# aifoundry-org/MHAQ

Hardware: AMD Instinct MI355X
Metric: qat_images_per_sec (higher is better)
Workload: dtype f32; 1 GPU; ResNet-18 ImageNet-1k QAT step, AEWGS weights per-channel + STE activations, Sym-KL distillation from FP teacher, RAdam, synthetic 224x224, channels_last memory format; per_gpu_batch=250, global_batch=250, parallelism=dp1, sync_batchnorm=False, weight_backward_groups=3, cudnn_benchmark=False

## Files before the change

include/mhaq_fq.h:

```cpp
#ifndef MHAQ_FQ_H
#define MHAQ_FQ_H

#include <stddef.h>
#include <stdint.h>

#ifdef __cplusplus
extern "C" {
#endif

#define MHAQ_FQ_ABI_VERSION 4

enum { MHAQ_FQ_STE = 0, MHAQ_FQ_EWGS = 1, MHAQ_FQ_AEWGS = 2, MHAQ_FQ_LSQ = 3 };

enum {
  MHAQ_FQ_EINVAL = -1,
  MHAQ_FQ_EWORKSPACE = -2,
  MHAQ_FQ_EALIGN = -3,
  MHAQ_FQ_EUNSUPPORTED = -4
};

enum {
  MHAQ_FQ_FLAG_BELOW_MIN = 1,
  MHAQ_FQ_FLAG_ABOVE_MAX = 2,
  MHAQ_FQ_FLAG_NOT_INTEGER = 4
// ... 70 lines not shown
                                  const float* params , int method, uint64_t seed, uint64_t offset,
                                  const uint64_t* offset_dev, void* workspace, size_t workspace_bytes,
                                  int32_t* nparts_out, void* stream);

int mhaq_fq_act_relu_fwd_x16(const void* z, const void* addend, void* y, void* a_out, int64_t n, int dtype,
                             const float* log_act_s, const float* log_act_q, const float* act_b,
                             float* params_out , void* stream);
int mhaq_fq_act_relu_bwd_x16(const void* z, const void* g_y, const void* g_a, void* gx, int64_t n, int dtype,
                             const float* params , int method, uint64_t seed, uint64_t offset,
                             const uint64_t* offset_dev, float* grads , void* workspace,
                             size_t workspace_bytes, void* stream);
int mhaq_fq_act_relu_bwd_partials_x16(const void* z, const void* g_y, const void* g_a, void* gx, int64_t n, int dtype,
                                      const float* params , int method, uint64_t seed, uint64_t offset,
                                      const uint64_t* offset_dev, void* workspace, size_t workspace_bytes,
                                      int32_t* nparts_out, void* stream);

size_t mhaq_fq_bn_bwd_workspace_bytes(int64_t m, int64_t c);
int mhaq_fq_bn_bwd(const float* x, const float* dy, const float* mean, const float* invstd, const float* weight,
                   float* dx, float* dweight, float* dbias, int64_t m, int64_t c,
                   void* workspace, size_t workspace_bytes, void* stream);

size_t mhaq_fq_bn_fwd_workspace_bytes(int64_t m, int64_t c);
int mhaq_fq_bn_fwd(const float* x, const float* weight, const float* bias, float* y,
                   float* save_mean, float* save_invstd, float* running_mean, float* running_var,
                   double factor, double eps, int64_t m, int64_t c,
                   void* workspace, size_t workspace_bytes, void* stream);

size_t mhaq_fq_bn_bwd_x16_workspace_bytes(int64_t m, int64_t c);
int mhaq_fq_bn_bwd_x16(const void* x, const void* dy, const float* mean, const float* invstd, const float* weight,
                       void* dx, float* dweight, float* dbias, int64_t m, int64_t c, int dtype,
                       void* workspace, size_t workspace_bytes, void* stream);

int mhaq_fq_maxpool3s2_fwd(const float* t, float* p, uint8_t* code, int64_t n, int64_t h, int64_t w, int64_t c,
                           void* stream);
size_t mhaq_fq_bn_pool_bwd_workspace_bytes(int64_t n, int64_t h, int64_t w, int64_t c);
int mhaq_fq_bn_pool_bwd(const float* x, const float* g, const uint8_t* code, const float* mean, const float* invstd,
                        const float* weight, float* dx, float* dweight, float* dbias, int64_t n, int64_t h, int64_t w,
                        int64_t c, void* workspace, size_t workspace_bytes, void* stream);

int mhaq_fq_maxpool3s2_fwd_x16(const void* t, void* p, uint8_t* code, int64_t n, int64_t h, int64_t w, int64_t c, int dtype,
                               void* stream);
size_t mhaq_fq_bn_pool_bwd_x16_workspace_bytes(int64_t n, int64_t h, int64_t w, int64_t c);
int mhaq_fq_bn_pool_bwd_x16(const void* x, const void* g, const uint8_t* code, const float* mean, const float* invstd,
                            const float* weight, void* dx, float* dweight, float* dbias, int64_t n, int64_t h, int64_t w,
                            int64_t c, int dtype, void* workspace, size_t workspace_bytes, void* stream);

enum { MHAQ_FQ_BN_RELU = 0, MHAQ_FQ_BN_ADD_RELU = 1, MHAQ_FQ_BN2_ADD_RELU = 2 };
int mhaq_fq_bn_infer_consts(const float* running_mean, const float* running_var, const float* weight, const float* bias,
                            double eps, int64_t c, float* consts , void* stream);
int mhaq_fq_bn_infer_act(const float* x, const float* consts, const float* x2, const float* consts2, const float* residual,
                         float* y, int64_t m, int64_t c, int mode, void* stream);
int mhaq_fq_bn_relu_pool3s2(const float* x, const float* consts, float* p, int64_t n, int64_t h, int64_t w, int64_t c,
                            void* stream);

size_t mhaq_fq_minmax_workspace_bytes(int64_t n);
int mhaq_fq_minmax(const float* x, int64_t n, float* out ,
                   void* workspace, size_t workspace_bytes, void* stream);

int mhaq_fq_row_minmax(const float* w, int64_t co, int64_t row, float* mn_out ,
                       float* mx_out , void* stream);

int mhaq_fq_pt_tie_scatter(const float* w, float* gw, int64_t n, const float* zp,
                           const float* grads , void* stream);

size_t mhaq_fq_pt_aewgs_colstats_workspace_bytes(int64_t co, int64_t row);
int mhaq_fq_pt_aewgs_colstats(const float* w, const float* G, int64_t co, int64_t row,
                              const float* s, const float* zp, const float* lo, const float* hi,
                              float* stats, void* workspace, size_t workspace_bytes, void* stream);

int mhaq_fq_pc_fwd(const float* w, float* wq, float* zp_out , float* q_out ,
                   const float* s , int64_t co, int64_t row, void* stream);

int mhaq_fq_pc_bwd(const float* w, const float* G, float* gw, float* g_s ,
                   const float* s , const float* zp ,
                   int64_t co, int64_t row, int method, const float* stats,
                   const float* gzp_extra ,
                   const int8_t* r_sign, uint64_t seed, uint64_t offset, const uint64_t* offset_dev, void* stream);

int mhaq_fq_wlayer_fwd(const float* w, float* wq, const float* log_s , int64_t co, int64_t row,
                       float* s_out, float* zp_out, float* mx_out, float* lwq_out ,
                       void* stream);
int mhaq_fq_wlayer_bwd(const float* w, const float* G, float* gw, float* g_log_s ,
                       const float* s, const float* zp, const float* mx, const float* g_lwq ,
                       int64_t co, int64_t row, int method, const float* stats,
                       const float* gzp_extra, const int8_t* r_sign, uint64_t seed, uint64_t offset, const uint64_t* offset_dev,
                       void* stream);

int64_t mhaq_fq_wlayer_pt_max_elements(void);
int mhaq_fq_wlayer_pt_fwd(const float* w, float* wq, const float* log_s , int64_t n,
                          float* aux , void* stream);
int mhaq_fq_wlayer_pt_bwd(const float* w, const float* G, float* gw, float* g_log_s ,
                          const float* aux, const float* g_lwq, int64_t n, int method,
                          const int8_t* r_sign, uint64_t seed, uint64_t offset, const uint64_t* offset_dev, void* stream);

size_t mhaq_fq_wlayer_ptl_workspace_bytes(int64_t n);
int mhaq_fq_wlayer_ptl_fwd(const float* w, float* wq, const float* log_s , int64_t n, float* aux ,
                           void* workspace, size_t workspace_bytes, void* stream);
int mhaq_fq_wlayer_ptl_bwd(const float* w, const float* G, float* gw, float* g_log_s ,
                           const float* aux , const float* g_lwq , int64_t n, int method,
                           const float* col_stats, int64_t period,
                           const int8_t* r_sign, uint64_t seed, uint64_t offset, const uint64_t* offset_dev,
                           void* workspace, size_t workspace_bytes, void* stream);

typedef struct {
  const float* w;
  const float* log_s;
// ... 58 lines not shown
```

mhaq_amd/_lib.py:

```python
from __future__ import annotations

import ctypes as C
import os
import re

_HERE = os.path.dirname(os.path.abspath(__file__))
LIB_PATH = os.environ.get("MHAQ_FQ_LIB") or os.path.join(_HERE, "csrc", "libmhaq_fq.so")
HEADER_PATH = os.path.join(os.path.dirname(_HERE), "include", "mhaq_fq.h")

_p = C.c_void_p
_i64 = C.c_int64
_u64 = C.c_uint64
_sz = C.c_size_t
_int = C.c_int

DT_BF16 = 1
DT_F16 = 2

SIGNATURES = {
    "mhaq_fq_abi_version": (_int, []),
    "mhaq_fq_error_string": (C.c_char_p, [_int]),
    "mhaq_fq_fill_r": (_int, [_p, _i64, _u64, _u64, _p]),
    "mhaq_fq_pt_fwd_workspace_bytes": (_sz, [_i64]),
    "mhaq_fq_pt_fwd": (_int, [_p, _p, _i64, _p, _p, _p, _p, _p, _p, _p, _p, _sz, _p]),
    "mhaq_fq_pt_bwd_workspace_bytes": (_sz, [_i64]),
    "mhaq_fq_pt_bwd": (_int, [_p, _p, _p, _i64, _p, _p, _p, _p, _int, _p, _i64, _p, _u64, _u64, _p, _int, _p, _p, _sz, _p]),
    "mhaq_fq_pt_bwd_partials": (_int, [_p, _p, _p, _i64, _p, _p, _p, _p, _int, _p, _i64, _p, _u64, _u64, _p, _int, _p, _sz,
                                       _p, _p]),
    "mhaq_fq_pt_bwd_finalize": (_int, [_p, C.c_int32, _p, _p]),
    "mhaq_fq_act_fwd": (_int, [_p, _p, _i64, _p, _p, _p, _p, _p, _p, _p, _sz, _p]),
    "mhaq_fq_act_bwd_workspace_bytes": (_sz, [_i64]),
    "mhaq_fq_act_bwd": (_int, [_p, _p, _p, _i64, _p, _int, _p, _u64, _u64, _p, _p, _p, _sz, _p]),
    "mhaq_fq_act_bwd_partials": (_int, [_p, _p, _p, _i64, _p, _int, _p, _u64, _u64, _p, _p, _sz, _p, _p]),
    "mhaq_fq_act_bwd_finalize_multi": (_int, [_p, _int, _p, _p]),
    "mhaq_fq_act_fwd_x16": (_int, [_p, _p, _i64, _int, _p, _p, _p, _p, _p, _p, _p, _sz, _p]),
    "mhaq_fq_act_bwd_x16": (_int, [_p, _p, _p, _i64, _int, _p, _int, _p, _u64, _u64, _p, _p, _p, _sz, _p]),
    "mhaq_fq_act_bwd_partials_x16": (_int, [_p, _p, _p, _i64, _int, _p, _int, _p, _u64, _u64, _p, _p, _sz, _p, _p]),
    "mhaq_fq_act_relu_fwd": (_int, [_p, _p, _p, _p, _i64, _p, _p, _p, _p, _p]),
    "mhaq_fq_act_relu_bwd": (_int, [_p, _p, _p, _p, _i64, _p, _int, _u64, _u64, _p, _p, _p, _sz, _p]),
    "mhaq_fq_act_relu_bwd_partials": (_int, [_p, _p, _p, _p, _i64, _p, _int, _u64, _u64, _p, _p, _sz, _p, _p]),
    "mhaq_fq_act_relu_fwd_x16": (_int, [_p, _p, _p, _p, _i64, _int, _p, _p, _p, _p, _p]),
    "mhaq_fq_act_relu_bwd_x16": (_int, [_p, _p, _p, _p, _i64, _int, _p, _int, _u64, _u64, _p, _p, _p, _sz, _p]),
    "mhaq_fq_act_relu_bwd_partials_x16": (_int, [_p, _p, _p, _p, _i64, _int, _p, _int, _u64, _u64, _p, _p, _sz, _p, _p]),
    "mhaq_fq_bn_bwd_workspace_bytes": (_sz, [_i64, _i64]),
    "mhaq_fq_bn_bwd": (_int, [_p, _p, _p, _p, _p, _p, _p, _p, _i64, _i64, _p, _sz, _p]),
    "mhaq_fq_bn_fwd_workspace_bytes": (_sz, [_i64, _i64]),
    "mhaq_fq_bn_fwd": (_int, [_p, _p, _p, _p, _p, _p, _p, _p, C.c_double, C.c_double, _i64, _i64, _p, _sz, _p]),
    "mhaq_fq_bn_bwd_x16_workspace_bytes": (_sz, [_i64, _i64]),
    "mhaq_fq_bn_bwd_x16": (_int, [_p, _p, _p, _p, _p, _p, _p, _p, _i64, _i64, _int, _p, _sz, _p]),
    "mhaq_fq_maxpool3s2_fwd": (_int, [_p, _p, _p, _i64, _i64, _i64, _i64, _p]),
    "mhaq_fq_bn_pool_bwd_workspace_bytes": (_sz, [_i64, _i64, _i64, _i64]),
    "mhaq_fq_bn_pool_bwd": (_int, [_p, _p, _p, _p, _p, _p, _p, _p, _p, _i64, _i64, _i64, _i64, _p, _sz, _p]),
    "mhaq_fq_maxpool3s2_fwd_x16": (_int, [_p, _p, _p, _i64, _i64, _i64, _i64, _int, _p]),
    "mhaq_fq_bn_pool_bwd_x16_workspace_bytes": (_sz, [_i64, _i64, _i64, _i64]),
    "mhaq_fq_bn_pool_bwd_x16": (_int, [_p, _p, _p, _p, _p, _p, _p, _p, _p, _i64, _i64, _i64, _i64, _int, _p, _sz, _p]),
    "mhaq_fq_bn_infer_consts": (_int, [_p, _p, _p, _p, C.c_double, _i64, _p, _p]),
    "mhaq_fq_bn_infer_act": (_int, [_p, _p, _p, _p, _p, _p, _i64, _i64, _int, _p]),
    "mhaq_fq_bn_relu_pool3s2": (_int, [_p, _p, _p, _i64, _i64, _i64, _i64, _p]),
    "mhaq_fq_minmax_workspace_bytes": (_sz, [_i64]),
    "mhaq_fq_minmax": (_int, [_p, _i64, _p, _p, _sz, _p]),
    "mhaq_fq_row_minmax": (_int, [_p, _i64, _i64, _p, _p, _p]),
    "mhaq_fq_pt_tie_scatter": (_int, [_p, _p, _i64, _p, _p, _p]),
    "mhaq_fq_pt_aewgs_colstats_workspace_bytes": (C.c_size_t, [_i64, _i64]),
    "mhaq_fq_pt_aewgs_colstats": (_int, [_p, _p, _i64, _i64, _p, _p, _p, _p, _p, _p, C.c_size_t, _p]),
    "mhaq_fq_pc_fwd": (_int, [_p, _p, _p, _p, _p, _i64, _i64, _p]),
    "mhaq_fq_pc_bwd": (_int, [_p, _p, _p, _p, _p, _p, _i64, _i64, _int, _p, _p, _p, _u64, _u64, _p, _p]),
    "mhaq_fq_pc_aewgs_stats": (_int, [_p, _p, _p, _p, _i64, _i64, _p, _p]),
    "mhaq_fq_wlayer_fwd": (_int, [_p, _p, _p, _i64, _i64, _p, _p, _p, _p, _p]),
    "mhaq_fq_wlayer_bwd": (_int, [_p, _p, _p, _p, _p, _p, _p, _p, _i64, _i64, _int, _p, _p, _p, _u64, _u64, _p, _p]),
    "mhaq_fq_wlayer_fwd_multi": (_int, [_p, _int, _i64, _i64, _p, _p, _p]),
    "mhaq_fq_wlayer_bwd_multi": (_int, [_p, _int, _i64, _i64, _p, _p, _p, _int, _p, _u64, _u64, _p, _p]),
    "mhaq_fq_wlayer_bwd_group": (_int, [_p, _int, _i64, _i64, _p, _i64, _p, _p, _int, _p, _u64, _u64, _p, _p]),
    "mhaq_fq_wlayer_aewgs_stats_group": (_int, [_p, _int, _i64, _p, _i64, _p, _p]),
    "mhaq_fq_pc_quantize": (_int, [_p, _p, _p, _p, _p, _i64, _i64, _p, _p]),
    "mhaq_fq_wlayer_pt_max_elements": (_i64, []),
    "mhaq_fq_wlayer_pt_fwd": (_int, [_p, _p, _p, _i64, _p, _p]),
    "mhaq_fq_wlayer_pt_bwd": (_int, [_p, _p, _p, _p, _p, _p, _i64, _int, _p, _u64, _u64, _p, _p]),
    "mhaq_fq_wlayer_ptl_workspace_bytes": (_sz, [_i64]),
    "mhaq_fq_wlayer_ptl_fwd": (_int, [_p, _p, _p, _i64, _p, _p, _sz, _p]),
    "mhaq_fq_wlayer_ptl_bwd": (_int, [_p, _p, _p, _p, _p, _p, _i64, _int, _p, _i64, _p, _u64, _u64, _p, _p, _sz, _p]),
    "mhaq_fq_vec_fwd": (_int, [_p, _p, _p, _p, _p, _i64, _p]),
    "mhaq_fq_vec_aewgs_stats": (_int, [_p, _p, _p, _p, _i64, _p, _p]),
    "mhaq_fq_vec_bwd": (_int, [_p, _p, _p, _p, _p, _p, _p, _i64, _int, _p, _p, _u64, _u64, _p, _p]),
    "mhaq_fq_potential_loss_fwd": (_int, [_p, _p, _p, _i64, _p, _p, _i64, C.c_float, C.c_float, C.c_float, _int,
                                          _p, _int, _p, _p]),
    "mhaq_fq_potential_loss_bwd": (_int, [_p, _p, _p, _p, _i64, _p, _p, _i64, C.c_float, C.c_float, C.c_float,
                                          _p, _p, _p, _p, _p, _p]),
    "mhaq_fq_noise_fwd": (_int, [_p, _p, _i64, _p]),
    "mhaq_fq_noise_bwd_workspace_bytes": (_sz, [_i64, _i64]),
    "mhaq_fq_noise_bwd": (_int, [_p, _p, _p, _p, _i64, _i64, _int, _p, _i64, _p, _u64, _u64, _p, _p, _sz, _p]),
}

_lib = None


class MhaqFqError(RuntimeError):
    pass


def header_functions():
    with open(HEADER_PATH) as f:
        src = re.sub(r"/\*.*?\*/", "", f.read(), flags=re.S)
    return sorted(set(re.findall(r"\b(mhaq_fq_\w+)\s*\(", src)))


def _try_build() -> None:
    import fcntl
    import subprocess
    import sys
    csrc = os.path.dirname(LIB_PATH)
    with open(os.path.join(csrc, ".build.lock"), "w") as lock:
# ... 37 lines not shown
```

mhaq_amd/csrc/torch_binding.cpp:

```cpp
#include <torch/extension.h>
#include <torch/version.h>
#include <torch/csrc/autograd/custom_function.h>

#include <c10/hip/HIPCachingAllocator.h>
#include <c10/hip/HIPGraphsC10Utils.h>
#include <c10/hip/HIPStream.h>
#include <c10/core/DeviceGuard.h>
#include <dlfcn.h>

#include <algorithm>
#include <atomic>
#include <chrono>
#include <cstring>
#include <map>
#include <memory>
#include <mutex>
#include <string>
#include <unordered_map>
#include <vector>

#include "../../include/mhaq_fq.h"

namespace py = pybind11;
using at::Tensor;
using torch::autograd::AutogradContext;
using torch::autograd::variable_list;

namespace {

#define MHAQ_API(X)                                                                                                   \
  X(mhaq_fq_abi_version) X(mhaq_fq_error_string) X(mhaq_fq_act_fwd) X(mhaq_fq_act_bwd_workspace_bytes)                \
  X(mhaq_fq_act_bwd) X(mhaq_fq_act_bwd_partials) X(mhaq_fq_act_bwd_finalize_multi) X(mhaq_fq_wlayer_fwd)              \
  X(mhaq_fq_wlayer_bwd) X(mhaq_fq_pc_aewgs_stats) X(mhaq_fq_wlayer_fwd_multi) X(mhaq_fq_wlayer_bwd_group)             \
  X(mhaq_fq_wlayer_aewgs_stats_group) X(mhaq_fq_wlayer_pt_fwd) X(mhaq_fq_wlayer_pt_bwd)                               \
  X(mhaq_fq_potential_loss_fwd) X(mhaq_fq_potential_loss_bwd) X(mhaq_fq_wlayer_ptl_workspace_bytes)                   \
  X(mhaq_fq_wlayer_ptl_fwd) X(mhaq_fq_wlayer_ptl_bwd) X(mhaq_fq_pt_aewgs_colstats_workspace_bytes)                     \
  X(mhaq_fq_pt_aewgs_colstats) X(mhaq_fq_act_fwd_x16) X(mhaq_fq_act_bwd_x16) X(mhaq_fq_act_bwd_partials_x16)                    \
  X(mhaq_fq_act_relu_fwd) X(mhaq_fq_act_relu_bwd) X(mhaq_fq_act_relu_bwd_partials)                                    \
  X(mhaq_fq_act_relu_fwd_x16) X(mhaq_fq_act_relu_bwd_x16) X(mhaq_fq_act_relu_bwd_partials_x16)                        \
  X(mhaq_fq_bn_bwd_workspace_bytes) X(mhaq_fq_bn_bwd) X(mhaq_fq_maxpool3s2_fwd)                                       \
  X(mhaq_fq_bn_pool_bwd_workspace_bytes) X(mhaq_fq_bn_pool_bwd) X(mhaq_fq_bn_bwd_x16_workspace_bytes)                 \
  X(mhaq_fq_bn_bwd_x16) X(mhaq_fq_bn_fwd_workspace_bytes) X(mhaq_fq_bn_fwd)                                         \
  X(mhaq_fq_bn_infer_consts) X(mhaq_fq_bn_infer_act) X(mhaq_fq_bn_relu_pool3s2)

struct Api {
#define X(n) decltype(&::n) n = nullptr;
  MHAQ_API(X)
#undef X
  void* handle = nullptr;
  std::string path;
};
Api A;

struct MhaqError : std::runtime_error {
  using std::runtime_error::runtime_error;
};

void bind_library(const std::string& path) {
  if (A.handle && A.path == path) return;
  void* h = dlopen(path.c_str(), RTLD_NOW | RTLD_LOCAL);
  if (!h) throw MhaqError("cannot load " + path + ": " + dlerror() + " (there is no CPU fallback)");
  Api a;
#define X(n)                                                                        \
  a.n = reinterpret_cast<decltype(a.n)>(dlsym(h, #n));                              \
  if (!a.n) throw MhaqError(std::string(#n) + " is not exported by " + path);
  MHAQ_API(X)
#undef X
  if (a.mhaq_fq_abi_version() != MHAQ_FQ_ABI_VERSION) throw MhaqError("libmhaq_fq.so ABI version mismatch");
  a.handle = h;
  a.path = path;
  A = a;
}

inline void need_lib() {
  if (!A.handle) throw MhaqError("the C-ABI library is not bound (mhaq_amd._ext.bind)");
}

inline void check(int rc, const char* what) {
  if (rc != 0)
    throw MhaqError(std::string(what) + " failed: " + A.mhaq_fq_error_string(rc) + " (code " + std::to_string(rc) + ")");
}

inline void* cur_stream(const Tensor& t) {
  return (void*)c10::hip::getCurrentHIPStream(t.device().index()).stream();
}

inline bool capturing() {
  return c10::hip::currentStreamCaptureStatusMayInitCtx() != c10::hip::CaptureStatus::None;
}

#define MHAQ_ON_DEVICE_OF(t) const c10::OptionalDeviceGuard mhaq_device_guard_(at::device_of(t))

inline const float* fptr(const Tensor& t) { return static_cast<const float*>(t.const_data_ptr()); }
inline float* fptr_mut(const Tensor& t) { return static_cast<float*>(t.mutable_data_ptr()); }
inline const float* fptr_or_null(const Tensor& t) { return t.defined() ? fptr(t) : nullptr; }

// ... 1267 lines not shown
    Tensor lws = lws_in.reshape({-1}).contiguous(), lwq = lwq_in.reshape({-1}).contiguous();
    TORCH_CHECK(las.numel() == laq.numel() && lws.numel() == lwq.numel(),
                "potential_loss: scale and range vectors must pair up");
    Tensor out = at::empty({12}, base.options());
    check(A.mhaq_fq_potential_loss_fwd(fptr(base), fptr(las), fptr(laq), las.numel(), fptr(lws), fptr(lwq), lws.numel(),
                                       (float)a_bits, (float)w_bits, (float)p, lossless ? 1 : 0, fptr_mut(state),
                                       update_state ? 1 : 0, fptr_mut(out), cur_stream(base)),
          "mhaq_fq_potential_loss_fwd");
    ctx->save_for_backward({out, las, laq, lws, lwq});
    ctx->saved_data["a"] = a_bits;
    ctx->saved_data["w"] = w_bits;
    ctx->saved_data["p"] = p;
    ctx->mark_non_differentiable({out});
    return {out.select(0, 0).clone(), out};
  }

  static variable_list backward(AutogradContext* ctx, variable_list grads) {
    auto saved = ctx->get_saved_variables();
    const Tensor &out = saved[0], &las = saved[1], &laq = saved[2], &lws = saved[3], &lwq = saved[4];
    Tensor g = grads[0].reshape({1}).contiguous();
    const int64_t na = las.numel(), nw = lws.numel();
    Tensor slab = at::empty({1 + 2 * na + 2 * nw}, out.options());
    Tensor g_base = slab.narrow(0, 0, 1), g_las = slab.narrow(0, 1, na), g_laq = slab.narrow(0, 1 + na, na),
           g_lws = slab.narrow(0, 1 + 2 * na, nw), g_lwq = slab.narrow(0, 1 + 2 * na + nw, nw);
    check(A.mhaq_fq_potential_loss_bwd(fptr(g), fptr(out), fptr(las), fptr(laq), na, fptr(lws), fptr(lwq), nw,
                                       (float)ctx->saved_data["a"].toDouble(), (float)ctx->saved_data["w"].toDouble(),
                                       (float)ctx->saved_data["p"].toDouble(), fptr_mut(g_base), fptr_mut(g_las),
                                       fptr_mut(g_laq), fptr_mut(g_lws), fptr_mut(g_lwq), cur_stream(out)),
          "mhaq_fq_potential_loss_bwd");
    const auto shapes = ctx->saved_data["shapes"].to<std::vector<std::vector<int64_t>>>();
    variable_list res(11);
    res[0] = g_base.reshape(shapes[0]);
    res[1] = g_las.reshape(shapes[1]);
    res[2] = g_laq.reshape(shapes[2]);
    res[3] = g_lws.reshape(shapes[3]);
    res[4] = g_lwq.reshape(shapes[4]);
    return res;
  }
};

std::pair<Tensor, Tensor> potential_loss(const Tensor& base, const Tensor& las, const Tensor& laq, const Tensor& lws,
                                         const Tensor& lwq, const Tensor& state, double a_bits, double w_bits, double p,
                                         bool lossless, bool update_state) {
  need_lib();
  MHAQ_ON_DEVICE_OF(base);
  for (const Tensor* t : {&base, &las, &laq, &lws, &lwq})
    TORCH_CHECK(t->is_cuda() && t->scalar_type() == at::kFloat, "potential_loss: inputs must be float32 device tensors");
  TORCH_CHECK(state.is_cuda() && state.scalar_type() == at::kFloat && state.numel() == 3 && state.is_contiguous(),
              "potential_loss: state must be a contiguous float32 device tensor {loss_sum, cnt, t}");
  auto out = PotentialLossFn::apply(base, las, laq, lws, lwq, state, a_bits, w_bits, p, lossless, update_state);
  return {out[0], out[1]};
}

}

PYBIND11_MODULE(TORCH_EXTENSION_NAME, m) {
  m.doc() = "compiled autograd binding of the mhaq_amd fused layer ops over the C ABI of include/mhaq_fq.h";
  m.attr("TORCH_VERSION") = TORCH_VERSION;
  static PyObject* err_class = nullptr;
  py::register_exception_translator([](std::exception_ptr p) {
    try {
      if (p) std::rethrow_exception(p);
    } catch (const MhaqError& e) {
      PyErr_SetString(err_class ? err_class : PyExc_RuntimeError, e.what());
    }
  });
  m.def("bind", [](const std::string& path, py::object error_class) {
    if (!err_class) err_class = error_class.inc_ref().ptr();
    bind_library(path);
  }, "dlopen the C-ABI library and resolve the entry points the nodes call");
  m.def("host_timers", [](bool reset) {
    py::dict d;
    for (int i = 0; i < T_N; ++i) {
      const int64_t n = g_tcnt[i].load(), ns = g_tns[i].load();
      d[kTimerNames[i]] = py::make_tuple(n, n ? (double)ns / (double)n * 1e-3 : 0.0);
      if (reset) { g_tcnt[i].store(0); g_tns[i].store(0); }
    }
    return d;
  }, py::arg("reset") = true);
  m.def("bound_library", []() { return A.path; });

  m.def("rng_manual_seed", [](uint64_t seed) { std::lock_guard<std::mutex> g(R.mu); R.seed = seed; R.seeded = true; R.count = 0; });
  m.def("rng_seed", []() -> py::object { std::lock_guard<std::mutex> g(R.mu); return R.seeded ? py::object(py::int_(R.seed)) : py::none(); });
  m.def("rng_next", [](int64_t rank) {
    std::lock_guard<std::mutex> g(R.mu);
    if (!R.seeded) throw MhaqError("sign stream used before it was seeded");
    return std::make_pair(R.seed ^ ((uint64_t)rank * kGolden), ++R.count);
  });
  m.def("rng_drawn", []() { std::lock_guard<std::mutex> g(R.mu); return R.count; });
  m.def("rng_set_drawn", [](uint64_t n) { std::lock_guard<std::mutex> g(R.mu); R.count = n; });
  m.def("rng_set_base", [](const std::optional<Tensor>& base) {
    std::lock_guard<std::mutex> g(R.mu);
    R.base = (base.has_value() && base->defined()) ? *base : Tensor();
  });
  m.def("rng_base", []() -> std::optional<Tensor> {
    std::lock_guard<std::mutex> g(R.mu);
    return R.base.defined() ? std::optional<Tensor>(R.base) : std::nullopt;
  });

  m.def("set_allreduce_avg", [](py::object fn) {
    g_allreduce_avg = fn.is_none() ? nullptr : fn.inc_ref().ptr();
  });
  m.def("set_dist_active", [](bool v) { g_dist_active.store(v); });

  m.def("hub_create", &hub_create);
  m.def("hub_destroy", [](int64_t id) { g_hubs.erase(id); });
// ... 33 lines not shown
        "number of BatchNorm backwards so far that ran the 16-bit HIP kernels (mhaq_fq_bn_bwd_x16)");
  m.def("bn_pool_train", &bn_pool_train, py::arg("x"), py::arg("weight"), py::arg("bias"), py::arg("running_mean"),
        py::arg("running_var"), py::arg("momentum"), py::arg("eps"), py::arg("cudnn_enabled") = true,
        py::arg("hip_forward") = false);
  m.def("bn_pool_hip_backwards", []() { return g_bn_pool_hip_backwards.load(); },
        "number of BatchNorm + pool backwards so far that ran mhaq_fq_bn_pool_bwd (the fallback is the two separate nodes)");

  m.def("bn_infer_consts", &bn_infer_consts, py::arg("running_mean"), py::arg("running_var"), py::arg("weight"),
        py::arg("bias"), py::arg("eps"), py::arg("consts"));
  m.def("bn_infer_act", &bn_infer_act, py::arg("x"), py::arg("consts"), py::arg("mode"), py::arg("x2") = py::none(),
        py::arg("consts2") = py::none(), py::arg("residual") = py::none());
  m.def("bn_relu_pool", &bn_relu_pool, py::arg("x"), py::arg("consts"));
  m.def("teacher_fused_calls", []() { return g_teacher_fused_calls.load(); },
        "number of fused launches so far on a frozen network's elementwise chain (bn_infer_act and bn_relu_pool)");

  m.def("weight_layer", &weight_layer, py::arg("w"), py::arg("log_wght_s"), py::arg("method"),
        py::arg("r_sign") = py::none(), py::arg("zp_grad") = false, py::arg("pre") = py::none(), py::arg("rank") = 0);
  m.def("weight_layer_pt", &weight_layer_pt, py::arg("w"), py::arg("log_wght_s"), py::arg("method"),
        py::arg("r_sign") = py::none(), py::arg("rank") = 0);
  m.def("weight_layer_ptl", &weight_layer_ptl, py::arg("w"), py::arg("log_wght_s"), py::arg("method"),
        py::arg("r_sign") = py::none(), py::arg("rank") = 0);

  m.def("plan_create", &plan_create);
  m.def("plan_destroy", [](int64_t id) { g_plans.erase(id); });
  m.def("plan_forward", &plan_forward);
  m.def("plan_group_apply", &plan_group_apply);
  m.def("plan_release_captured", [](int64_t id) {
    auto p = g_plans.get(id);
    std::lock_guard<std::mutex> g(p->mu);
    for (auto& grp : p->groups) if (grp.pool) grp.pool->release_captured();
    p->fwd_tables.release_captured();
  });
  m.def("plan_state", [](int64_t id) {
    auto p = g_plans.get(id);
    std::lock_guard<std::mutex> g(p->mu);
    py::dict d;
    d["fwd_tables"] = p->fwd_tables.entries.size();
    py::list pools;
    for (auto& grp : p->groups) {
      py::dict e;
      size_t used = 0, held = 0, size = 0;
      if (grp.pool) {
        size = grp.pool->keys.size();
        for (size_t i = 0; i < size; ++i) { used += grp.pool->used[i]; held += grp.pool->held[i]; }
      }
      e["size"] = size; e["used"] = used; e["held"] = held;
      pools.append(e);
    }
    d["pools"] = pools;
    return d;
  });

  m.def("potential_loss", &potential_loss);
}
```

mhaq_amd/qat.py:

```python
from __future__ import annotations

import contextlib
import copy
import time
from dataclasses import dataclass, field
from typing import Optional

import torch
import torch.distributed as dist
from torch import nn

from . import ops
from ._lib import MhaqFqError
from .enums import QNMethod, QScheme
from .loss import FusedPotentialLoss, FusedPotentialLossNoPred, SymmetricalKL
from .wrap import get_model_values, quantize_model


@dataclass
class QATConfig:
    qscheme: QScheme = QScheme.PER_CHANNEL
    qnmethod: QNMethod = QNMethod.AEWGS
    act_bit: int = 1
    weight_bit: int = 1
    calib_act_bit: int = 10
    calib_weight_bit: int = 10
    excluded_layers: tuple = ("conv1", "fc")
    quantize_bias: bool = False
    distillation: bool = True
    learning_rate: float = 3e-4
    warmup: int = 100
    scale_lr: float = 1.0
    scale_t: float = 2.0
    sync_batchnorm: bool = True
    overlap_teacher: bool = True
    joint_act_finalize: bool = True
    student_high_priority: bool = False
    multi_weight_forward: bool = True
    weight_backward_group_elems: int = 4 << 20
    fuse_blocks: bool = True
    fuse_stem_pool: bool = True
    hip_bn_backward: bool = True
    hip_bn_backward_16bit: bool = False
    hip_bn_forward: bool = False
    fuse_teacher: bool = True
    criterion: nn.Module = field(default_factory=nn.CrossEntropyLoss)
    autocast_dtype: Optional[torch.dtype] = None


@torch.no_grad()
def calibrate_weights(model: nn.Module, wbits: int, max_bits: int = 24, row_minmax_fn=None) -> None:
    row_minmax_fn = row_minmax_fn or ops.row_minmax
    for m in model.modules():
        if hasattr(m, "log_wght_s") and hasattr(m, "weight"):
            mn, mx = row_minmax_fn(m.weight)
            mn, mx = mn.cpu(), mx.cpu()
            if m.log_wght_s.numel() == 1 and mn.numel() != 1:
                mn, mx = mn.min(), mx.max()
            if not m.log_wght_s.requires_grad:
                wbits = max_bits
            floor = torch.log2((mx - mn) / (2 ** wbits - 1)).reshape(m.log_wght_s.shape)
            m.log_wght_s.copy_(torch.max(m.log_wght_s.detach().cpu(), floor))


def _cpu_row_minmax(w):
    dims = tuple(range(1, w.dim()))
    return w.detach().amin(dims), w.detach().amax(dims)


@torch.no_grad()
def calibrate_activations(model: nn.Module, batches, abits: int, max_bits: int = 24, minmax_fn=None) -> None:
    minmax_fn = minmax_fn or ops.minmax
    acts = [m for m in model.modules() if hasattr(m, "log_act_s") and hasattr(m, "act_b")]
    seen = {id(a): [] for a in acts}
    hooks = [a.register_forward_pre_hook(lambda mod, inp: seen[id(mod)].append(minmax_fn(inp[0]))) for a in acts]
    was_training = model.training
    model.eval()
    for x in batches:
        model(x)
    for h in hooks:
        h.remove()
    model.train(was_training)
    for a in acts:
        mm = torch.stack(seen[id(a)]).cpu()
        mn, mx = mm[:, 0].min(), mm[:, 1].max()
        if not a.log_act_q.requires_grad and not a.log_act_s.requires_grad:
            abits = max_bits
        if mx - mn > 0:
            log_s = torch.log2((mx - mn) / (2 ** abits - 1))
            a.act_b.fill_(mn)
            a.log_act_s.fill_(log_s)
            a.log_act_q.fill_(log_s + abits)
        else:
            a.log_act_q.zero_(), a.log_act_s.zero_(), a.act_b.fill_(mn)
            a.log_act_q.requires_grad_(False), a.log_act_s.requires_grad_(False), a.act_b.requires_grad_(False)


class TemperatureSchedule:
# ... 112 lines not shown
                pass
        self.module = _QATModule(net, cfg.qscheme, self.act_hub, self.weight_forward)
        self._flat_sync = False
        want_capture = capture_graph
        if want_capture is None:
            want_capture = "auto" if (layers is None and optimizer_factory is None and not multi_tensor_weights) else False
        if self.distributed and want_capture and self.device.type == "cuda" and self.multi is None:
            step_collectives = any(isinstance(m, nn.SyncBatchNorm) for m in net.modules()) or any(
                ops._method_value(m.Q.qnmethod) == QNMethod.AEWGS.value for m in net.modules() if hasattr(m, "Q")
            ) or next(iter(net.buffers()), None) is not None
            self._flat_sync = not step_collectives
        if self.distributed:
            for p in [m.log_b_s for m in net.modules() if hasattr(m, "log_b_s")]:
                p.requires_grad_(False)
            if self._flat_sync:
                with torch.no_grad():
                    for t in list(net.parameters()) + list(net.buffers()):
                        dist.broadcast(t, 0)
            else:
                self._wrap_ddp()
        if loss_classes is None:
            if self.device.type != "cuda":
                raise MhaqFqError("QATTrainer on a CPU device needs loss_classes (and layers): the fake-quant path and "
                                  "its PotentialLoss run only as HIP kernels (no CPU fallback by design)")
            loss_classes = (FusedPotentialLoss, FusedPotentialLossNoPred)
        if cfg.distillation:
            self.loss = loss_classes[0](SymmetricalKL(), p=1, a=cfg.act_bit, w=cfg.weight_bit)
        else:
            self.loss = loss_classes[1](cfg.criterion, p=1, a=cfg.act_bit, w=cfg.weight_bit)
        if capture_graph is None:
            stock = layers is None and optimizer_factory is None and not multi_tensor_weights
            capture_graph = "auto" if stock else False
        self.capture_graph = capture_graph if capture_graph == "auto" else bool(capture_graph)
        self._graph = self._static = self._static_loss = None
        self._rng_base = None
        self._rng_host0 = self._rng_stride = 0
        self._preflight, self._preflight_syncs = False, []
        self._flat_cache = None
        self._eager_steps = 0
        self._host_share = []
        self._static_grads, self._grads_detached = [], False
        if self.capture_graph:
            if (self.distributed and not self._flat_sync) or self.device.type != "cuda" or self.multi is not None:
                if self.capture_graph == "auto":
                    self.capture_graph = False
                else:
                    raise ValueError("capture_graph needs a step without host code or collectives inside it: a "
                                     "single GPU, or data parallelism without SyncBatchNorm and without the AEWGS "
                                     "statistics exchange (then the gradients take one flat all-reduce after the "
                                     "replay); not the multi-tensor joint backward")
        if self.capture_graph:
            self._rng_base = torch.zeros(1, dtype=torch.int64, device=self.device)
            self._gstream = torch.cuda.Stream(device=self.device)
        self.optimizer = (optimizer_factory or torch.optim.RAdam)(self.net.parameters(), cfg.learning_rate)
        self.schedule = TemperatureSchedule(cfg.learning_rate, cfg.warmup, cfg.scale_lr, cfg.scale_t)
        self.schedule.start(self.optimizer)

    def _autocast(self):
        if self.cfg.autocast_dtype is None:
            return contextlib.nullcontext()
        return torch.autocast(self.device.type, dtype=self.cfg.autocast_dtype, cache_enabled=False)

    def _wrap_ddp(self):
        ids = [self.device.index] if self.device.type == "cuda" else None
        self.module = nn.parallel.DistributedDataParallel(self.module, device_ids=ids, find_unused_parameters=False,
                                                          gradient_as_bucket_view=True)
        self._flat_sync = False

    def _agree(self, *flags):
        if not self.distributed:
            return tuple(bool(f) for f in flags)
        v = torch.tensor([1.0 if f else 0.0 for f in flags], dtype=torch.float32, device=self.device)
        dist.all_reduce(v, op=dist.ReduceOp.MAX)
        return tuple(x > 0.5 for x in v.tolist())

    def _step_is_gpu_bound(self) -> bool:
        return min(self._host_share[1:]) < 0.8

    @staticmethod
    def _flat_alias(g):
        if not ops._is_dense(g):
            raise MhaqFqError("flat gradient all-reduce: a gradient is not dense")
        return g.as_strided((g.numel(),), (1,), g.storage_offset())

    def _sync_grads(self, static=False):
        cache = self._flat_cache if static else None
        if cache is None:
            grads = [p.grad for p in self.net.parameters() if p.grad is not None]
            views = [self._flat_alias(g) for g in grads]
            flat = torch.empty(sum(v.numel() for v in views), dtype=torch.float32, device=self.device)
            cache = (views, flat, list(flat.split([v.numel() for v in views])))
            if static:
                self._flat_cache = cache
        views, flat, parts = cache
        torch.cat(views, out=flat)
        ops._allreduce_avg_(flat)
        torch._foreach_copy_(views, parts)

    def train_step(self, x, y):
        if not self.capture_graph:
            if self._hp_stream is not None:
                cur = torch.cuda.current_stream()
                self._hp_stream.wait_stream(cur)
                with torch.cuda.stream(self._hp_stream):
                    loss = self._step(x, y)
                cur.wait_stream(self._hp_stream)
            else:
# ... 198 lines not shown
```

Before: 6694 images/s.

## Replace foreach RAdam with a single fused HIP kernel over all parameters

Adds a HIP kernel that runs the whole RAdam update (moments, rectification, parameter step) in one launch across all parameter tensors. It uses a chunked work table and a cached device descriptor table, and the step-dependent scalars are computed on the host. QAT training switches to this optimizer by default on GPU. The aim is to replace the many foreach kernel launches and repeated passes over memory with one read-modify-write pass. In exchange, the host now calls .item() on every step tensor, which may synchronise, and the kernel rules out graph capture.

```diff
diff --git a/include/mhaq_fq.h b/include/mhaq_fq.h
--- a/include/mhaq_fq.h
+++ b/include/mhaq_fq.h
@@ -146,6 +146,22 @@
                          float* y, int64_t m, int64_t c, int mode, void* stream);
 int mhaq_fq_bn_relu_pool3s2(const float* x, const float* consts, float* p, int64_t n, int64_t h, int64_t w, int64_t c,
                             void* stream);
+
+typedef struct {
+  float* p;
+  const float* g;
+  float* m;
+  float* v;
+  int64_t n;
+  float c1, c2;
+} mhaq_radam_desc;
+typedef struct {
+  int32_t tensor;
+  int32_t chunk;
+} mhaq_radam_work;
+int64_t mhaq_fq_radam_chunk_elements(void);
+int mhaq_fq_radam_step(const mhaq_radam_desc* descs_device, int ntensors, const mhaq_radam_work* work_device,
+                       int64_t nwork, float w1, float beta2, float w2, float eps, void* stream);
 
 size_t mhaq_fq_minmax_workspace_bytes(int64_t n);
 int mhaq_fq_minmax(const float* x, int64_t n, float* out ,
diff --git a/mhaq_amd/_lib.py b/mhaq_amd/_lib.py
--- a/mhaq_amd/_lib.py
+++ b/mhaq_amd/_lib.py
@@ -57,6 +57,8 @@
     "mhaq_fq_bn_infer_consts": (_int, [_p, _p, _p, _p, C.c_double, _i64, _p, _p]),
     "mhaq_fq_bn_infer_act": (_int, [_p, _p, _p, _p, _p, _p, _i64, _i64, _int, _p]),
     "mhaq_fq_bn_relu_pool3s2": (_int, [_p, _p, _p, _i64, _i64, _i64, _i64, _p]),
+    "mhaq_fq_radam_chunk_elements": (_i64, []),
+    "mhaq_fq_radam_step": (_int, [_p, _int, _p, _i64, C.c_float, C.c_float, C.c_float, C.c_float, _p]),
     "mhaq_fq_minmax_workspace_bytes": (_sz, [_i64]),
     "mhaq_fq_minmax": (_int, [_p, _i64, _p, _p, _sz, _p]),
     "mhaq_fq_row_minmax": (_int, [_p, _i64, _i64, _p, _p, _p]),
diff --git a/mhaq_amd/csrc/optim.hip b/mhaq_amd/csrc/optim.hip
--- /dev/null
+++ b/mhaq_amd/csrc/optim.hip
@@ -0,0 +1,140 @@
+#include <hip/hip_runtime.h>
+
+#include "../../include/mhaq_fq.h"
+#include "fq_common.hpp"
+
+#ifndef MHAQ_RADAM_FORM
+#define MHAQ_RADAM_FORM 7
+#endif
+#ifndef MHAQ_RADAM_G_NT
+#define MHAQ_RADAM_G_NT 1
+#endif
+#ifndef MHAQ_RADAM_LD_NT
+#define MHAQ_RADAM_LD_NT 1
+#endif
+#ifndef MHAQ_RADAM_ST_NT
+#define MHAQ_RADAM_ST_NT 0
+#endif
+
+namespace mhaq {
+
+constexpr int kRadamForm = MHAQ_RADAM_FORM;
+constexpr bool kRadamGNt = MHAQ_RADAM_G_NT != 0, kRadamLdNt = MHAQ_RADAM_LD_NT != 0, kRadamStNt = MHAQ_RADAM_ST_NT != 0;
+constexpr int kRadamU = 4;
+constexpr int kRadamChunk = kBlock * 4 * kRadamU;
+
+struct RadamK {
+  float w1, beta2, w2, eps, one, c1, c2;
+};
+
+__device__ __forceinline__ void radam_element(float& p, float g, float& m, float& v, const RadamK& k) {
+  const float d = g - m;
+  if (fabsf(k.w1) < 0.5f) {
+    m = (kRadamForm & 1) ? fmaf(k.w1, d, m) : m + k.w1 * d;
+  } else {
+    const float u = 1.0f - k.w1;
+    m = (kRadamForm & 1) ? fmaf(-d, u, g) : g - d * u;
+  }
+  v = v * k.beta2;
+  float a, b;
+  if (kRadamForm & 8) { a = k.w2 * g; b = g; } else { a = k.w2; b = g * g; }
+  v = (kRadamForm & 2) ? fmaf(a, b, v) : v + a * b;
+  float t = sqrtf(v);
+  t = t + k.eps;
+  t = t / k.c2;
+  t = 1.0f / t;
+  t = t + k.c1;
+  const float mt = m * t;
+  p = (kRadamForm & 4) ? fmaf(k.one, mt, p) : p + mt;
+}
+
+template <bool NT>
+__device__ __forceinline__ vf4 radam_ld4(const float* q) {
+  const vf4 MHAQ_GLOBAL_AS* a = gptr(reinterpret_cast<const vf4*>(q));
+  return NT ? __builtin_nontemporal_load(a) : *a;
+}
+__device__ __forceinline__ void radam_st4(float* q, vf4 x) {
+  vf4 MHAQ_GLOBAL_AS* a = gptr(reinterpret_cast<vf4*>(q));
+  if constexpr (kRadamStNt) __builtin_nontemporal_store(x, a);
+  else *a = x;
+}
+
+__global__ __launch_bounds__(kBlock) void radam_step_kernel(const mhaq_radam_desc* __restrict__ descs, int ntensors,
+                                                            const mhaq_radam_work* __restrict__ work, float w1,
+                                                            float beta2, float w2, float eps, float one) {
+  const mhaq_radam_work wk = work[blockIdx.x];
+  if (wk.tensor < 0 || wk.tensor >= ntensors || wk.chunk < 0) return;
+  const mhaq_radam_desc t = descs[wk.tensor];
+  const int64_t e0 = (int64_t)wk.chunk * kRadamChunk;
+  if (e0 >= t.n) return;
+  const int len = (int)(t.n - e0 < kRadamChunk ? t.n - e0 : kRadamChunk);
+  float* __restrict__ p = t.p + e0;
+  const float* __restrict__ g = t.g + e0;
+  float* __restrict__ m = t.m + e0;
+  float* __restrict__ v = t.v + e0;
+  const RadamK k{w1, beta2, w2, eps, one, t.c1, t.c2};
+  const int tid = (int)threadIdx.x;
+  if ((((uintptr_t)p | (uintptr_t)g | (uintptr_t)m | (uintptr_t)v) & 15) == 0) {
+    const int nv = len >> 2;
+    vf4 vp[kRadamU], vg[kRadamU], vm[kRadamU], vv[kRadamU];
+#pragma unroll
+    for (int u = 0; u < kRadamU; ++u) {
+      const int i = tid + u * kBlock;
+      if (i < nv) {
+        vg[u] = radam_ld4<kRadamGNt>(g + 4 * i);
+        vm[u] = radam_ld4<kRadamLdNt>(m + 4 * i);
+        vv[u] = radam_ld4<kRadamLdNt>(v + 4 * i);
+        vp[u] = radam_ld4<kRadamLdNt>(p + 4 * i);
+      }
+    }
+#pragma unroll
+    for (int u = 0; u < kRadamU; ++u) {
+      const int i = tid + u * kBlock;
+      if (i < nv) {
+#pragma unroll
+        for (int j = 0; j < 4; ++j) {
+          float pj = vp[u][j], mj = vm[u][j], vj = vv[u][j];
+          radam_element(pj, vg[u][j], mj, vj, k);
+          vp[u][j] = pj; vm[u][j] = mj; vv[u][j] = vj;
+        }
+        radam_st4(m + 4 * i, vm[u]);
+        radam_st4(v + 4 * i, vv[u]);
+        radam_st4(p + 4 * i, vp[u]);
+      }
+    }
+    const int i = (nv << 2) + tid;
+    if (i < len) {
+      float pj = ldg(p + i), mj = ldg(m + i), vj = ldg(v + i);
+      radam_element(pj, ldg(g + i), mj, vj, k);
+      stg(m + i, mj); stg(v + i, vj); stg(p + i, pj);
+    }
+  } else {
+    for (int i = tid; i < len; i += kBlock) {
+      float pj = ldg(p + i), mj = ldg(m + i), vj = ldg(v + i);
+      radam_element(pj, ldg(g + i), mj, vj, k);
+      stg(m + i, mj); stg(v + i, vj); stg(p + i, pj);
+    }
+  }
+}
+
+}
+
+using namespace mhaq;
+
+extern "C" {
+
+int64_t mhaq_fq_radam_chunk_elements(void) { return kRadamChunk; }
+
+int mhaq_fq_radam_step(const mhaq_radam_desc* descs_device, int ntensors, const mhaq_radam_work* work_device,
+                       int64_t nwork, float w1, float beta2, float w2, float eps, void* stream) {
+  if (ntensors < 0 || nwork < 0) return MHAQ_FQ_EINVAL;
+  if (nwork == 0) return 0;
+  if (!descs_device || !work_device || ntensors == 0) return MHAQ_FQ_EINVAL;
+  if (nwork > 0x7fffffff) return MHAQ_FQ_EUNSUPPORTED;
+  if (((uintptr_t)descs_device & 7) || ((uintptr_t)work_device & 7)) return MHAQ_FQ_EALIGN;
+  MHAQ_LAUNCH(radam_step_kernel, dim3((unsigned)nwork), dim3(kBlock), 0, (hipStream_t)stream, descs_device, ntensors,
+              work_device, w1, beta2, w2, eps, 1.0f );
+  return launch_status();
+}
+
+}
diff --git a/mhaq_amd/csrc/torch_binding.cpp b/mhaq_amd/csrc/torch_binding.cpp
--- a/mhaq_amd/csrc/torch_binding.cpp
+++ b/mhaq_amd/csrc/torch_binding.cpp
@@ -41,7 +41,8 @@
   X(mhaq_fq_bn_bwd_workspace_bytes) X(mhaq_fq_bn_bwd) X(mhaq_fq_maxpool3s2_fwd)                                       \
   X(mhaq_fq_bn_pool_bwd_workspace_bytes) X(mhaq_fq_bn_pool_bwd) X(mhaq_fq_bn_bwd_x16_workspace_bytes)                 \
   X(mhaq_fq_bn_bwd_x16) X(mhaq_fq_bn_fwd_workspace_bytes) X(mhaq_fq_bn_fwd)                                         \
-  X(mhaq_fq_bn_infer_consts) X(mhaq_fq_bn_infer_act) X(mhaq_fq_bn_relu_pool3s2)
+  X(mhaq_fq_bn_infer_consts) X(mhaq_fq_bn_infer_act) X(mhaq_fq_bn_relu_pool3s2)                                     \
+  X(mhaq_fq_radam_chunk_elements) X(mhaq_fq_radam_step)
 
 struct Api {
 #define X(n) decltype(&::n) n = nullptr;
@@ -1415,6 +1416,92 @@
   return {out[0], out[1]};
 }
 
+struct RadamTables {
+  std::mutex mu;
+  std::map<std::pair<int, int64_t>, std::unique_ptr<TablePool>> descs;
+  std::map<int, TableCache> work;
+  static constexpr size_t kWorkLists = 4;
+  static constexpr int64_t kDescGrain = 64;
+};
+RadamTables& g_radam = *new RadamTables();
+std::atomic<int64_t> g_fused_radam_steps{0};
+
+bool same_memory_order(const Tensor& a, const Tensor& b) {
+  if (a.sizes() != b.sizes()) return false;
+  for (int64_t d = 0; d < a.dim(); ++d)
+    if (a.size(d) != 1 && a.stride(d) != b.stride(d)) return false;
+  return true;
+}
+
+void radam_step(const std::vector<Tensor>& params, const std::vector<Tensor>& grads, const std::vector<Tensor>& exp_avgs,
+                const std::vector<Tensor>& exp_avg_sqs, const std::vector<double>& c1s, const std::vector<double>& c2s,
+                double beta1, double beta2, double eps) {
+  need_lib();
+  const size_t n = params.size();
+  TORCH_CHECK(grads.size() == n && exp_avgs.size() == n && exp_avg_sqs.size() == n && c1s.size() == n && c2s.size() == n,
+              "radam_step: the six lists must have one length");
+  if (n == 0) return;
+  TORCH_CHECK(!capturing(), "radam_step: a captured launch would freeze the step-dependent scalars; step eagerly");
+  const Tensor& like = params[0];
+  TORCH_CHECK(like.is_cuda(), "radam_step: device tensors are required (there is no CPU path)");
+  for (size_t i = 0; i < n; ++i) {
+    const Tensor& p = params[i];
+    for (const Tensor* t : {&p, &grads[i], &exp_avgs[i], &exp_avg_sqs[i]})
+      TORCH_CHECK(t->defined() && t->device() == like.device() && t->scalar_type() == at::kFloat &&
+                      t->is_non_overlapping_and_dense() && same_memory_order(*t, p),
+                  "radam_step: tensor ", i, ": p, grad, exp_avg and exp_avg_sq must be dense float32 tensors on one device "
+                  "in the same memory order");
+  }
+  MHAQ_ON_DEVICE_OF(like);
+  void* st = cur_stream(like);
+  const int dev = (int)like.device().index();
+  const int64_t chunk = A.mhaq_fq_radam_chunk_elements();
+  std::vector<mhaq_radam_desc> descs(n);
+  std::vector<int64_t> key, sizes;
+  key.reserve(6 * n);
+  sizes.reserve(n);
+  int64_t nwork = 0;
+  for (size_t i = 0; i < n; ++i) {
+    mhaq_radam_desc& d = descs[i];
+    d.p = fptr_mut(params[i]);
+    d.g = fptr(grads[i]);
+    d.m = fptr_mut(exp_avgs[i]);
+    d.v = fptr_mut(exp_avg_sqs[i]);
+    d.n = params[i].numel();
+    d.c1 = (float)c1s[i];
+    d.c2 = (float)c2s[i];
+    int64_t scalars;
+    static_assert(sizeof(scalars) == 2 * sizeof(float), "two floats per key word");
+    std::memcpy(&scalars, &d.c1, sizeof(scalars));
+    for (int64_t w : {(int64_t)(uintptr_t)d.p, (int64_t)(uintptr_t)d.g, (int64_t)(uintptr_t)d.m, (int64_t)(uintptr_t)d.v,
+                      d.n, scalars})
+      key.push_back(w);
+    sizes.push_back(d.n);
+    nwork += (d.n + chunk - 1) / chunk;
+  }
+  if (nwork == 0) return;
+  std::lock_guard<std::mutex> guard(g_radam.mu);
+  const int64_t cap = ((int64_t)n + RadamTables::kDescGrain - 1) / RadamTables::kDescGrain * RadamTables::kDescGrain;
+  auto& pool = g_radam.descs[{dev, cap}];
+  if (!pool) pool = std::make_unique<TablePool>(sizeof(mhaq_radam_desc) * (size_t)cap, like);
+  const Tensor& dtab = pool->get(key, [&](void* host) {
+    std::memset(host, 0, sizeof(mhaq_radam_desc) * (size_t)cap);
+    std::memcpy(host, descs.data(), sizeof(mhaq_radam_desc) * n);
+  }, st);
+  const Tensor wtab = g_radam.work[dev].get(sizes, RadamTables::kWorkLists, like, [&]() {
+    std::vector<mhaq_radam_work> w;
+    w.reserve((size_t)nwork);
+    for (size_t i = 0; i < n; ++i)
+      for (int64_t c = 0; c * chunk < sizes[i]; ++c) w.push_back({(int32_t)i, (int32_t)c});
+    return w;
+  });
+  check(A.mhaq_fq_radam_step(static_cast<const mhaq_radam_desc*>(dtab.const_data_ptr()), (int)n,
+                             static_cast<const mhaq_radam_work*>(wtab.const_data_ptr()), nwork, (float)(1.0 - beta1),
+                             (float)beta2, (float)(1.0 - beta2), (float)eps, st),
+        "mhaq_fq_radam_step");
+  g_fused_radam_steps.fetch_add(1, std::memory_order_relaxed);
+}
+
 }
 
 PYBIND11_MODULE(TORCH_EXTENSION_NAME, m) {
@@ -1554,4 +1641,9 @@
   });
 
   m.def("potential_loss", &potential_loss);
-}
+  m.def("radam_step", &radam_step, py::arg("params"), py::arg("grads"), py::arg("exp_avgs"), py::arg("exp_avg_sqs"),
+        py::arg("c1s"), py::arg("c2s"), py::arg("beta1"), py::arg("beta2"), py::arg("eps"),
+        "one launch of mhaq_fq_radam_step over the listed tensors (mhaq_amd/optim.py)");
+  m.def("fused_radam_steps", []() { return g_fused_radam_steps.load(); },
+        "launches of mhaq_fq_radam_step so far (tests: the optimizer step took the HIP kernel)");
+}
diff --git a/mhaq_amd/optim.py b/mhaq_amd/optim.py
--- /dev/null
+++ b/mhaq_amd/optim.py
@@ -0,0 +1,155 @@
+from __future__ import annotations
+
+import os
+
+import torch
+from torch.optim.optimizer import _use_grad_for_differentiable
+from torch.optim.radam import _multi_tensor_radam, radam as _radam
+
+ENV_SWITCH = "MHAQ_FUSED_RADAM"
+
+_fallbacks = 0
+
+
+def enabled(configured: bool = True) -> bool:
+    v = os.environ.get(ENV_SWITCH)
+    if v is None or not v.strip():
+        return bool(configured)
+    return v.strip().lower() in ("1", "true", "on", "yes")
+
+
+def fused_radam_steps() -> int:
+    from . import _ext
+    return int(_ext.ext().fused_radam_steps())
+
+
+def fused_radam_fallbacks() -> int:
+    return _fallbacks
+
+
+def radam_scalars(step: float, lr: float, beta1: float, beta2: float):
+    rho_inf = 2 / (1 - beta2) - 1
+    rho_t = rho_inf - 2 * step * (beta2 ** step) / (1 - beta2 ** step)
+    rect = (((rho_t - 4) * (rho_t - 2) * rho_inf / ((rho_inf - 4) * (rho_inf - 2) * rho_t)) ** 0.5
+            if rho_t > 5 else 0)
+    unrectified = 0 if rect > 0 else 1.0
+    bias_correction1 = 1 - beta1 ** step
+    c1 = (lr * unrectified / bias_correction1) * -1
+    c2 = ((1 - beta2 ** step) ** 0.5) * (lr * rect / bias_correction1) * -1
+    return c1, c2
+
+
+def group_fallback_reason(group):
+    if group["weight_decay"] != 0:
+        return "weight_decay"
+    for flag in ("maximize", "capturable", "differentiable"):
+        if group.get(flag, False):
+            return flag
+    if type(group["lr"]) is not float:
+        return "lr"
+    return None
+
+
+def _memory_order(t):
+    return tuple((n, s) for n, s in zip(t.shape, t.stride()) if n != 1)
+
+
+def _dense(order) -> bool:
+    expect = 1
+    for n, s in sorted(order, key=lambda ns: ns[1]):
+        if s != expect:
+            return False
+        expect *= n
+    return True
+
+
+_dense_orders = {}
+
+
+def tensor_fallback_reason(p, g, m, v, require_gpu: bool = True):
+    ts = (p, g, m, v)
+    for t in ts:
+        if t.dtype is not torch.float32:
+            return "dtype"
+    dev = p.device
+    if (require_gpu and dev.type != "cuda") or g.device != dev or m.device != dev or v.device != dev:
+        return "device"
+    for t in ts:
+        if t.layout is not torch.strided:
+            return "layout"
+    order = _memory_order(p)
+    if not (p.shape == g.shape == m.shape == v.shape) or not (order == _memory_order(g) == _memory_order(m)
+                                                              == _memory_order(v)):
+        return "order"
+    ok = _dense_orders.get(order)
+    if ok is None:
+        if len(_dense_orders) > 4096:
+            _dense_orders.clear()
+        ok = _dense_orders[order] = p.numel() == 0 or _dense(order)
+    return None if ok else "dense"
+
+
+class FusedRAdam(torch.optim.RAdam):
+
+    _one = None
+
+    @_use_grad_for_differentiable
+    def step(self, closure=None):
+        global _fallbacks
+        self._cuda_graph_capture_health_check()
+        loss = None
+        if closure is not None:
+            with torch.enable_grad():
+                loss = closure()
+        for group in self.param_groups:
+            params, grads, exp_avgs, exp_avg_sqs, steps = [], [], [], [], []
+            beta1, beta2 = group["betas"]
+            has_complex = self._init_group(group, params, grads, exp_avgs, exp_avg_sqs, steps)
+            if not params:
+                continue
+            if group_fallback_reason(group) is None:
+                rest = [i for i in range(len(params))
+                        if tensor_fallback_reason(params[i], grads[i], exp_avgs[i], exp_avg_sqs[i]) is not None]
+            else:
+                rest = list(range(len(params)))
+            if rest:
+                _fallbacks += len(rest)
+                pick = lambda xs: [xs[i] for i in rest]
+                kw = dict(beta1=beta1, beta2=beta2, lr=group["lr"], weight_decay=group["weight_decay"], eps=group["eps"],
+                          decoupled_weight_decay=group["decoupled_weight_decay"], differentiable=group["differentiable"],
+                          maximize=group["maximize"], capturable=group["capturable"], has_complex=has_complex)
+                lists = (pick(params), pick(grads), pick(exp_avgs), pick(exp_avg_sqs), pick(steps))
+                if group["differentiable"]:
+                    _radam(*lists, foreach=False, **kw)
+                else:
+                    _multi_tensor_radam(*lists, **kw)
+                if len(rest) == len(params):
+                    continue
+                skip = set(rest)
+                keep = [i for i in range(len(params)) if i not in skip]
+                params, grads, exp_avgs, exp_avg_sqs, steps = ([xs[i] for i in keep]
+                                                               for xs in (params, grads, exp_avgs, exp_avg_sqs, steps))
+            self._fused(group, params, grads, exp_avgs, exp_avg_sqs, steps, beta1, beta2)
+        return loss
+
+    def _fused(self, group, params, grads, exp_avgs, exp_avg_sqs, steps, beta1, beta2):
+        from . import _ext
+        if FusedRAdam._one is None:
+            FusedRAdam._one = torch.tensor(1.0, device="cpu")
+        torch._foreach_add_(steps, FusedRAdam._one, alpha=1.0)
+        lr = group["lr"]
+        memo, c1s, c2s = {}, [], []
+        for s in steps:
+            k = s.item()
+            c = memo.get(k)
+            if c is None:
+                c = memo[k] = radam_scalars(k, lr, beta1, beta2)
+            c1s.append(c[0])
+            c2s.append(c[1])
+        by_device = {}
+        for i, p in enumerate(params):
+            by_device.setdefault(p.device, []).append(i)
+        for idx in by_device.values():
+            pick = (lambda xs: xs) if len(idx) == len(params) else (lambda xs: [xs[i] for i in idx])
+            _ext.ext().radam_step(pick(params), pick(grads), pick(exp_avgs), pick(exp_avg_sqs), pick(c1s), pick(c2s),
+                                  beta1, beta2, group["eps"])
diff --git a/mhaq_amd/qat.py b/mhaq_amd/qat.py
--- a/mhaq_amd/qat.py
+++ b/mhaq_amd/qat.py
@@ -44,6 +44,7 @@
     hip_bn_backward_16bit: bool = False
     hip_bn_forward: bool = False
     fuse_teacher: bool = True
+    fused_optimizer: bool = True
     criterion: nn.Module = field(default_factory=nn.CrossEntropyLoss)
     autocast_dtype: Optional[torch.dtype] = None
 
@@ -262,7 +263,12 @@
         if self.capture_graph:
             self._rng_base = torch.zeros(1, dtype=torch.int64, device=self.device)
             self._gstream = torch.cuda.Stream(device=self.device)
-        self.optimizer = (optimizer_factory or torch.optim.RAdam)(self.net.parameters(), cfg.learning_rate)
+        make_optimizer = optimizer_factory or torch.optim.RAdam
+        if optimizer_factory is None and self.device.type == "cuda":
+            from . import optim
+            if optim.enabled(cfg.fused_optimizer):
+                make_optimizer = optim.FusedRAdam
+        self.optimizer = make_optimizer(self.net.parameters(), cfg.learning_rate)
         self.schedule = TemperatureSchedule(cfg.learning_rate, cfg.warmup, cfg.scale_lr, cfg.scale_t)
         self.schedule.start(self.optimizer)
 
```

Measured after the change: 6766 images/s, median of 6. 1.1% higher.
